# AlmondGod/diffusion-piano

Measured on AMD Instinct MI355X. Metric: env steps/sec at 4096 parallel envs; qpos L∞ drift vs CPU MuJoCo, higher is better.
Workload: dtype f32; 1 GPU; 4096 envs/GPU crossing_field random-action rollout, 10 physics substeps per env-step, constraint forces by the primal Newton solve (friction loss, uncapped rows); envs_per_gpu=4096, song=crossing_field, parallelism=dp1

## Files before the change

__graft_entry__.py:

```python

from __future__ import annotations

import importlib
import os
import subprocess
import sys
from pathlib import Path

ROOT = Path(__file__).resolve().parent
PKG = ROOT / "diffusion-piano_amd"
HIPCC = os.environ.get("HIPCC", "/opt/rocm/bin/hipcc")


_PENDING = []


def _hipcc(src_name, out_name, extra_deps=(), flags=(), wait=True):
    src = PKG / "csrc" / src_name
    out = PKG / out_name
    deps = [src, *extra_deps, Path(__file__)]
    if out.exists() and all(out.stat().st_mtime >= d.stat().st_mtime for d in deps):
        return out
    cmd = [HIPCC, "--offload-arch=gfx950", "-O3", "-std=c++17", "-fPIC", "-shared", "-Wno-unused-value", *flags,
           "-o", str(out), str(src)]
    if wait:
        subprocess.run(cmd, check=True)
    else:
        _PENDING.append((subprocess.Popen(cmd), cmd))
    return out


def _join():
    while _PENDING:
        proc, cmd = _PENDING.pop()
        if proc.wait() != 0:
            raise subprocess.CalledProcessError(proc.returncode, cmd)


def _hipcc_lib():
    csrc = PKG / "csrc"
    deps = [csrc / "devmodel.h", csrc / "prims.h", csrc / "collide_x.h", csrc / "kernel_v2.inc", csrc / "newton.inc",
            csrc / "augment.inc", csrc / "song_build.h", ROOT / "include" / "pianosim.h"]
    flags = ["-fno-hip-fp32-correctly-rounded-divide-sqrt", "-falign-loops=64", "-mllvm", "-amdgpu-sched-strategy=max-ilp"]
    out = _hipcc("pianosim.hip", "libpianosim.so", deps, flags=flags, wait=False)
    _hipcc("pianosim.hip", "libpianosim_timing.so", deps, flags=flags + ["-DPS_TIMING"], wait=False)
    return out


def _hipcc_xcheck():
    csrc = PKG / "csrc"
    src, out = ROOT / "tools" / "xcheck.hip", ROOT / "tools" / "libxcheck.so"
    deps = [src, csrc / "devmodel.h", csrc / "prims.h", csrc / "collide_x.h", ROOT / "include" / "pianosim.h"]
    if out.exists() and all(out.stat().st_mtime >= d.stat().st_mtime for d in deps):
        return out
    subprocess.run([HIPCC, "--offload-arch=gfx950", "-O3", "-std=c++17", "-fPIC", "-shared", "-Wno-unused-value",
                    "-fno-hip-fp32-correctly-rounded-divide-sqrt", "-o", str(out), str(src)], check=True)
    return out


def _hipcc_ldl_bench():
    src, out = ROOT / "tools" / "ldl_bench.hip", ROOT / "tools" / "libldlbench.so"
    if out.exists() and out.stat().st_mtime >= src.stat().st_mtime:
        return out
    subprocess.run([HIPCC, "--offload-arch=gfx950", "-O3", "-std=c++17", "-fPIC", "-shared", "-Wno-unused-value",
                    "-o", str(out), str(src)], check=True)
    return out


def _hipcc_rl():
    deps = [ROOT / "include" / "pianorl.h", PKG / "csrc" / "mlp_step.inc", PKG / "csrc" / "mlp_split.inc"]
    ilp = ["-mllvm", "-amdgpu-sched-strategy=max-ilp"]
    _hipcc("pianorl.hip", "libpianorl_timing.so", deps, flags=ilp + ["-DMLP_TIMING"], wait=False)
    return _hipcc("pianorl.hip", "libpianorl.so", deps, flags=ilp, wait=False)


def _gxx_song():
    src = PKG / "csrc" / "song.cpp"
    out = PKG / "libpianosong.so"
    deps = [src, PKG / "csrc" / "song_build.h", ROOT / "include" / "pianosong.h", Path(__file__)]
    if out.exists() and all(out.stat().st_mtime >= d.stat().st_mtime for d in deps):
        return out
    subprocess.run(["g++", "-O2", "-std=c++17", "-fPIC", "-shared", "-Wall", "-ffp-contract=off", "-o", str(out),
                    str(src)], check=True)
    return out


def build() -> None:
    _hipcc_lib()
    _hipcc_rl()
    _hipcc_xcheck()
    _hipcc_ldl_bench()
    _gxx_song()
    _join()
    subprocess.run(["make", "-s", "-C", str(ROOT / "oracle")], check=True)
    sys.path.insert(0, str(ROOT))
    pkg = importlib.import_module("diffusion-piano_amd")
    lib = importlib.import_module("diffusion-piano_amd._lib").load()
    assert lib.ps_model_desc_size() > 0
# ... 47 lines not shown
```

diffusion-piano_amd/csrc/kernel_v2.inc:

```

#ifdef PS_TIMING
#define NPHASE 56
#define TARG , uint64_t *tacc, uint64_t &tlast
#define TPASS , tacc, tlast
#define TSTAMP(slot)                                     \
  do {                                                   \
    __syncthreads();                                     \
    uint64_t t_ = __builtin_amdgcn_s_memtime();         \
    tacc[slot] += t_ - tlast;                            \
    tlast = t_;                                          \
  } while (0)
__device__ uint64_t* g_timing = nullptr;
#else
#define TSTAMP(slot) \
  do {               \
  } while (0)
#define TARG
#define TPASS
#endif

#ifdef PS_CHECK_A
__device__ int g_dbg_count = 0;
#endif
enum : int { BX_R = 0, BX_CP = 0, BX_O = 10, BX_W = 13, BX_AL = 16, BX_AC = 19, BX_F = 22, BX_N = 25, BXS = 28 };
// ... 1105 lines not shown
    float val;
    if (i < G) {
      int j = i / (NK + 1), k = i - j * (NK + 1);
      int t = t_obs + j;
      val = t < song.T ? song.goal[t * (NK + 1) + k] : 0.f;
    } else if (i < o_s) {
      int slot = i - o_f;
      val = 0.f;
      for (int n = 0; n < song.count[t_obs]; n++) {
        int f = song.fingers[t_obs * PS_MAX_NOTES + n];
        int idx = f < 5 ? (f < 0 ? f + 5 : f) : f;
        if (idx == slot) val = 1.f;
      }
    } else if (i < o_s + NK) {
      val = S.knorm[i - o_s];
    } else if (i == o_s + NK) {
      val = S.sustain;
    } else {
      val = S.dx[m->obs_dof[i - o_s - NK - 1]][6];
    }
    obs[i] = val;
  }
}

__device__ __forceinline__ void key_state2(const DevModel* __restrict__ m, Shared& S, const LaneDyn& D, int lane) {
  uint64_t bits[2];
#pragma unroll
  for (int j = 0; j < 2; j++) {
    int k = lane + 64 * j;
    bool act = false;
    if (k < NK) {
      float khi = m->key_hi[k];
      float s = clampf(D.kq[j], m->key_lo[k], khi);
      S.knorm[k] = s / khi;
      act = fabsf(s - khi) <= KEY_THRESHOLD;
    }
    bits[j] = __ballot(act);
  }
  if (lane == 0) {
    S.act_bits[0] = (int)(bits[0] & 0xffffffffull);
    S.act_bits[1] = (int)(bits[0] >> 32);
    S.act_bits[2] = (int)(bits[1] & 0xffffffull);
  }
  wsync();
}

#ifndef PS_BIG_SWEEPS
#define PS_BIG_SWEEPS 2
#endif
#ifndef PS_WAVES_PER_EU
#define PS_WAVES_PER_EU 2
#endif
#ifndef PS_CHUNKS
#define PS_CHUNKS 3
#endif
template <bool XG, int WPE, bool Q>
__device__ __forceinline__ bool env_step(Shared& S, const DevModel* __restrict__ m, const Song& songs, const Cfg& cfg,
                                         const Bufs& bufs, const float* __restrict__ action,
                                         const uint8_t* __restrict__ mask, float* __restrict__ obs,
                                         float* __restrict__ reward, float* __restrict__ discount,
                                         uint8_t* __restrict__ step_type, const int mode, const int e, const int lane,
                                         const int chunk, const int chunks) {
  const bool first = !Q || chunk == 0;
  const Song song = song_of(songs, e);
  float* obs_e = obs + (size_t)e * cfg.obs_dim;
  bool do_reset;
  if (mode == 1) {
    if (mask && !mask[e]) return false;
    do_reset = true;
  } else {
    do_reset = first && bufs.last[e] != 0;
  }
  const float* applied = bufs.applied ? bufs.applied + (size_t)e * NV : nullptr;
  const float* cw = bufs.park + (size_t)e * PARK_WORDS * 64 + lane;
  int cscal = 0;
  if (Q && !first) {
    cscal = __float_as_int(ld_wt(cw + 64 * CW_SCAL));
    if (__builtin_amdgcn_readlane(cscal, CS_NOAPPLIED)) applied = nullptr;
  }
  float hand_dy = 0.f;
  if (do_reset) {
    const int ep = bufs.episode[e];
    if (cfg.randomize) hand_dy = hand_offset_draw(cfg.seed_lo, cfg.seed_hi, (int)(cfg.env0 + (uint32_t)e), ep);
    if (lane == 0) {
      bufs.episode[e] = ep + 1;
      bufs.hand_dy[e] = hand_dy;
    }
  } else if (cfg.randomize) {
    hand_dy = bufs.hand_dy[e];
  }
  LaneStatic L;
  load_static(m, S, L, lane);
  LaneDyn D;
  const size_t rowoff = (size_t)e * NV;
  D.qws = 0.f;
#pragma unroll
  for (int j = 0; j < 2; j++) D.kws[j] = 0.f;
  if (do_reset) {
    D.q = D.v = 0.f;
    #pragma unroll
    for (int j = 0; j < 2; j++) { D.kq[j] = D.kv[j] = 0.f; }
    if (lane == 0) S.sustain = 0.f;
  } else if (Q && !first) {
    D.q = ld_wt(cw + 64 * CW_Q);
    D.v = ld_wt(cw + 64 * CW_V);
#pragma unroll
    for (int j = 0; j < 2; j++) {
// ... 23 lines not shown
    if (src < 0) ctrl = 0.f;
    if (Q && !first) ctrl = ld_wt(cw + 64 * CW_CTRL);
    const float sv = a_e[m->n_action - 1];
    if (lane == 0) S.sustain = cfg.canonical ? (sv + 1.f) * 0.5f : sv;
  }
  wsync();
  float actf_last = 0.f;
  int st_solves = 0, st_concap = 0, st_cap = 0, st_maxrow = 0, st_coupled = 0, st_piv = 0, st_cdofs = 0;
#ifdef PS_TIMING
  uint64_t tacc[NPHASE] = {0};
  uint64_t tlast = __builtin_amdgcn_s_memtime();
#endif
  int warn[PS_NWARN] = {0, 0, 0};
  if (Q && !first) {
    actf_last = ld_wt(cw + 64 * CW_ACTF);
    st_solves = __builtin_amdgcn_readlane(cscal, CS_SOLVES);
    st_concap = __builtin_amdgcn_readlane(cscal, CS_CONCAP);
    st_cap = __builtin_amdgcn_readlane(cscal, CS_CAP);
    st_maxrow = __builtin_amdgcn_readlane(cscal, CS_MAXROW);
    st_coupled = __builtin_amdgcn_readlane(cscal, CS_COUPLED);
    st_piv = __builtin_amdgcn_readlane(cscal, CS_PIV);
    st_cdofs = __builtin_amdgcn_readlane(cscal, CS_CDOFS);
    static_assert(PS_NWARN == 3, "carried warning counters");
    warn[0] = __builtin_amdgcn_readlane(cscal, CS_WARN);
    warn[1] = __builtin_amdgcn_readlane(cscal, CS_WARN + 1);
    warn[2] = __builtin_amdgcn_readlane(cscal, CS_WARN + 2);
  }
#define PS_RESET_PHYSICS()                                                              \
  do {                                                                                  \
    D.q = D.v = D.qws = 0.f;                                                            \
    for (int j_ = 0; j_ < 2; j_++) D.kq[j_] = D.kv[j_] = D.kws[j_] = 0.f;               \
    ctrl = 0.f;                                                                         \
    if (applied) {                                                                      \
      for (int i_ = lane; i_ < NV; i_ += 64) const_cast<float*>(applied)[i_] = 0.f;     \
      applied = nullptr;                                                                \
    }                                                                                   \
  } while (0)
  if (!do_reset) {
    bool acc_reset = false;
    NGuess guess;
    guess.zf = guess.zl = guess.zc = 0;
    guess.cid = -2;
    guess.zk[0] = guess.zk[1] = 0;
    guess.valid = false;
    if (Q && !first) {
      guess.zf = __float_as_int(ld_wt(cw + 64 * CW_ZF));
      guess.zl = __float_as_int(ld_wt(cw + 64 * CW_ZL));
      guess.zc = __float_as_int(ld_wt(cw + 64 * CW_ZC));
      guess.cid = __float_as_int(ld_wt(cw + 64 * CW_CID));
      guess.zk[0] = __float_as_int(ld_wt(cw + 64 * CW_ZK));
      guess.zk[1] = __float_as_int(ld_wt(cw + 64 * (CW_ZK + 1)));
      guess.valid = __builtin_amdgcn_readlane(cscal, CS_GVALID) != 0;
    }
    const int s_begin = Q ? chunk * m->nsub / chunks : 0;
    const int s_end = Q ? (chunk + 1) * m->nsub / chunks : m->nsub;
    for (int s = s_begin; s < (Q ? s_end : m->nsub); s++) {
      {
        bool bq = lane < NDT && !(fabsf(D.q) <= 1e10f), bv = false;
#pragma unroll
        for (int j = 0; j < 2; j++)
          if (lane + 64 * j < NK) bq |= !(fabsf(D.kq[j]) <= 1e10f);
        if (__ballot(bq)) { warn[PS_WARN_BADQPOS]++; PS_RESET_PHYSICS(); }
        bv = lane < NDT && !(fabsf(D.v) <= 1e10f);
#pragma unroll
        for (int j = 0; j < 2; j++)
          if (lane + 64 * j < NK) bv |= !(fabsf(D.kv[j]) <= 1e10f);
        if (__ballot(bv)) { warn[PS_WARN_BADQVEL]++; PS_RESET_PHYSICS(); }
      }
      int zoff = 0;
      asm volatile("" : "+s"(zoff));
      const DevModel* __restrict__ mq = m + zoff;
      int lq = lane;
      asm volatile("" : "+v"(lq));
      kinematics2<true, XG>(mq, S, L, D, lq, hand_dy TPASS);
      TSTAMP(0);
      D.actf = ctrl;
      dynamics2(mq, S, L, D, applied, lq TPASS);
      actf_last = D.w;
      TSTAMP(1);
      if (XG) {
        float* pkc = bufs.park + (size_t)e * PARK_WORDS * 64 + lq;
#pragma unroll
        for (int a = 0; a < MAXDEP; a++) {
          pkc[64 * a] = D.M[a];
          pkc[64 * (9 + a)] = D.Mh[a];
        }
        pkc[64 * 18] = D.q; pkc[64 * 19] = D.v; pkc[64 * 20] = D.qws; pkc[64 * 21] = D.qfs;
#pragma unroll
        for (int j = 0; j < 2; j++) {
          pkc[64 * (22 + j)] = D.kq[j];
          pkc[64 * (24 + j)] = D.kv[j];
          pkc[64 * (26 + j)] = D.kws[j];
          pkc[64 * (28 + j)] = D.kqfs[j];
        }
        asm volatile("" ::: "memory");
      }
      st_concap += collide2<XG, WPE>(mq, S, cfg.maxcon, lq, L.c_r TPASS) >= cfg.maxcon;
      if (XG) {
        asm volatile("" ::: "memory");
        const float* pkc = bufs.park + (size_t)e * PARK_WORDS * 64 + lq;
#pragma unroll
        for (int a = 0; a < MAXDEP; a++) {
          D.M[a] = pkc[64 * a];
          D.Mh[a] = pkc[64 * (9 + a)];
        }
        D.q = pkc[64 * 18]; D.v = pkc[64 * 19]; D.qws = pkc[64 * 20]; D.qfs = pkc[64 * 21];
#pragma unroll
        for (int j = 0; j < 2; j++) {
// ... 341 lines not shown
  if (lane == 0) {
    float* tm = bufs.terms + (size_t)e * PS_NTERMS;
    tm[0] = kp; tm[1] = sus; tm[2] = energy; tm[3] = fing; tm[4] = fore;
    reward[e] = kp + sus + energy + fing + fore;
    discount[e] = disc;
    step_type[e] = terminal ? PS_LAST : PS_MID;
    float* ma = bufs.mus_acc + (size_t)e * PS_NMUSIC;
#pragma unroll
    for (int i = 0; i < PS_NMUSIC; i++) ma[i] += mus[i];
    if (terminal) {
      float* me = bufs.mus_ep + (size_t)e * PS_NMUSIC;
      const float inv = 1.f / (float)t_new;
#pragma unroll
      for (int i = 0; i < PS_NMUSIC; i++) me[i] = ma[i] * inv;
      bufs.mus_cnt[e] += 1;
    }
    bufs.sustain[e] = S.sustain;
    bufs.t_idx[e] = t_new;
    bufs.last[e] = terminal ? 1 : 0;
    bufs.ncon[e] = S.ncon;
  }
  if (bufs.con_out) {
    constexpr int CW = (int)(sizeof(Contact) / sizeof(int));
    const int* src = reinterpret_cast<const int*>(S.con);
    int* dst = reinterpret_cast<int*>(bufs.con_out) + (size_t)e * MAXCON * CW;
    for (int w = lane; w < S.ncon * CW; w += 64) dst[w] = src[w];
  }
#ifdef PS_TIMING
  TSTAMP(5);
  if (lane == 0 && g_timing)
    for (int i = 0; i < NPHASE; i++) g_timing[(size_t)e * NPHASE + i] += tacc[i];
#endif
  return false;
}

template <bool XG, int WPE = PS_WAVES_PER_EU>
__global__ void __launch_bounds__(64) __attribute__((amdgpu_waves_per_eu(WPE))) pianosim_kernel(const DevModel* __restrict__ m, Song song, Cfg cfg, Bufs bufs,
                                                      const float* __restrict__ action, const uint8_t* __restrict__ mask,
                                                      float* __restrict__ obs, float* __restrict__ reward,
                                                      float* __restrict__ discount, uint8_t* __restrict__ step_type,
                                                      int mode, int n_envs, const int* __restrict__ order) {
#ifdef PS_DYN_LDS
  extern __shared__ __attribute__((aligned(16))) char smem_[];
  Shared& S = *reinterpret_cast<Shared*>(smem_);
#else
  __shared__ Shared S;
#endif
  const int e = order ? order[blockIdx.x] : (int)blockIdx.x;
  const int lane = threadIdx.x;
  if (e >= n_envs) return;
  env_step<XG, WPE, false>(S, m, song, cfg, bufs, action, mask, obs, reward, discount, step_type, mode, e, lane, 0, 1);
}

enum : int { QC_HEAD = 0, QC_TAIL = 32, QC_WORDS = 64 };
#ifndef PS_TIMING
enum : int { QE_NONE = -1, QE_LEFT = -2 };
struct QArgs {
  const DevModel* m;
  Song song;
  Cfg cfg;
  Bufs bufs;
  const float* action;
  float *obs, *reward, *discount;
  uint8_t* step_type;
  int n_envs;
  int *queue, *ctr;
  int cap, chunks;
};
template <bool XG>
__global__ void __launch_bounds__(64) __attribute__((amdgpu_waves_per_eu(PS_WAVES_PER_EU))) pianosim_queue_kernel(
    const QArgs ka) {
  __shared__ Shared S;
  typedef __attribute__((address_space(4))) const QArgs* KArgs;
  const uint64_t kbase = (uint64_t)__builtin_amdgcn_kernarg_segment_ptr();
  int own = ka.queue[blockIdx.x];
  for (;;) {
    int lane = threadIdx.x;
    asm volatile("" : "+v"(lane));
    uint64_t kp = kbase;
    asm volatile("" : "+s"(kp));
    const QArgs& a = *(const QArgs*)(KArgs)kp;
    int item = own;
    if (own < 0 && lane == 0) {
      const int t = __hip_atomic_fetch_add(&a.ctr[QC_HEAD], 1, __ATOMIC_RELAXED, __HIP_MEMORY_SCOPE_AGENT);
      if (t < a.cap) item = __hip_atomic_exchange(&a.queue[t], QE_LEFT, __ATOMIC_RELAXED, __HIP_MEMORY_SCOPE_AGENT);
      __builtin_amdgcn_fence(__ATOMIC_ACQUIRE, "agent");
    }
    asm volatile("s_waitcnt vmcnt(0)" ::: "memory");
    item = __builtin_amdgcn_readfirstlane(item);
    asm volatile("" : "+s"(item));
    wsync();
    if (item < 0) return;
    const int e = item >> 4, chunk = item & 15;
    if (e >= a.n_envs) return;
    const bool more = env_step<XG, PS_WAVES_PER_EU, true>(S, a.m, a.song, a.cfg, a.bufs, a.action, nullptr, a.obs, a.reward,
                                                          a.discount, a.step_type, 0, e, lane, chunk, a.chunks);
    asm volatile("s_waitcnt vmcnt(0)" ::: "memory");
    wsync();
    own = QE_NONE;
    if (more) {
      const int next = (e << 4) | (chunk + 1);
      int old = QE_NONE;
      if (lane == 0) {
        const int slot = __hip_atomic_fetch_add(&a.ctr[QC_TAIL], 1, __ATOMIC_RELAXED, __HIP_MEMORY_SCOPE_AGENT);
        old = slot < a.cap ? __hip_atomic_exchange(&a.queue[slot], next, __ATOMIC_RELAXED, __HIP_MEMORY_SCOPE_AGENT)
                           : (int)QE_LEFT;
      }
      if (__builtin_amdgcn_readfirstlane(old) == QE_LEFT) own = next;
    }
    wsync();
  }
}
#endif
```

diffusion-piano_amd/csrc/pianosim.hip:

```cpp
#include <hip/hip_runtime.h>
#include <math.h>
#include <stdint.h>
#include <stdio.h>
#include <stdlib.h>
#include <string.h>

#include <string>
#include <vector>

#include "devmodel.h"
#include "prims.h"
#include "collide_x.h"

using namespace ps;

#include "kernel_v2.inc"
#include "augment.inc"

static thread_local std::string g_err;
static int fail(const std::string& s) {
  g_err = s;
  return -1;
}
#define HIPCHK(x)                                                                    \
  do {                                                                               \
    hipError_t e_ = (x);                                                             \
    if (e_ != hipSuccess) return fail(std::string(#x) + ": " + hipGetErrorString(e_)); \
  } while (0)

struct ps_env {
  int n, device, obs_dim, action_dim;
  int64_t env_offset;
  int full_cpl;
  ps_task_cfg cfg;
  DevModel* d_model;
  int T;
  float* d_goal;
  int *d_count, *d_keys, *d_fingers;
  float *qpos, *qvel, *qws, *ctrl, *sustain, *applied, *terms, *tips;
  int *t_idx, *ncon;
  float *mus_acc, *mus_ep;
  int* mus_cnt;
  int* order;
  bool ordered;
  uint8_t* last;
  bool applied_on;
  float* hand_dy;
  int* episode;
  int* stats;
  int* warnings;
  float* park;
  uint64_t seed;
  bool has_x;
  int wave_slots;
  int chunks, step_grid;
  bool chunks_forced;
  int *queue, *qctr;
  Contact* con_out;
  bool aug_on;
  AugDev aug;
  size_t aug_lds;
  std::vector<void*> aug_mem;
};

struct DeviceGuard {
  int prev = -1;
  bool ok = true;
  explicit DeviceGuard(int dev) {
    if (hipGetDevice(&prev) != hipSuccess) prev = -1;
    if (prev != dev) ok = hipSetDevice(dev) == hipSuccess;
  }
  ~DeviceGuard() {
    int cur = -1;
    if (prev >= 0 && hipGetDevice(&cur) == hipSuccess && cur != prev) (void)hipSetDevice(prev);
  }
};
#define GUARD(E)                                                                  \
  DeviceGuard guard_((E)->device);                                                \
  if (!guard_.ok) return fail("hipSetDevice(" + std::to_string((E)->device) + ") failed")

static void quat2mat_h(const double* q, float* R) {
  double n = sqrt(q[0] * q[0] + q[1] * q[1] + q[2] * q[2] + q[3] * q[3]);
  double w = q[0] / n, x = q[1] / n, y = q[2] / n, z = q[3] / n;
  double M[9] = {1 - 2 * (y * y + z * z), 2 * (x * y - w * z), 2 * (x * z + w * y),
                 2 * (x * y + w * z), 1 - 2 * (x * x + z * z), 2 * (y * z - w * x),
                 2 * (x * z - w * y), 2 * (y * z + w * x), 1 - 2 * (x * x + y * y)};
  for (int i = 0; i < 9; i++) R[i] = (float)M[i];
}

static void enclosing_capsule(const double (*v)[3], int n, float* out) {
  double best = INFINITY;
  double lo[3] = {INFINITY, INFINITY, INFINITY}, hi[3] = {-INFINITY, -INFINITY, -INFINITY};
  for (int i = 0; i < n; i++)
    for (int k = 0; k < 3; k++) { lo[k] = fmin(lo[k], v[i][k]); hi[k] = fmax(hi[k], v[i][k]); }
  for (int a = 0; a < 3; a++) {
    const int b = (a + 1) % 3, c = (a + 2) % 3;
    const double cb = 0.5 * (lo[b] + hi[b]), cc = 0.5 * (lo[c] + hi[c]);
    double r = 0.0;
    for (int i = 0; i < n; i++) r = fmax(r, hypot(v[i][b] - cb, v[i][c] - cc));
    double t0 = INFINITY, t1 = -INFINITY;
    for (int i = 0; i < n; i++) {
      const double rho = hypot(v[i][b] - cb, v[i][c] - cc), s = sqrt(fmax(r * r - rho * rho, 0.0));
      t0 = fmin(t0, v[i][a] + s);
      t1 = fmax(t1, v[i][a] - s);
    }
    if (t0 > t1) t0 = t1 = 0.5 * (t0 + t1);
    const double vol = M_PI * r * r * (t1 - t0) + 4.0 / 3.0 * M_PI * r * r * r;
    if (vol < best) {
      best = vol;
      double p0[3], p1[3];
// ... 359 lines not shown
    for (int s = 0; s < PS_NFINGER; s++) {
      m->site_body[h * PS_NFINGER + s] = h * NB + d->site_body[h][s];
      for (int i = 0; i < 3; i++) m->site_pos[h * PS_NFINGER + s][i] = (float)d->site_pos[h][s][i];
    }
  if (d->n_cappairs < 0 || d->n_cappairs > PS_MAX_CAPPAIRS) return fail("bad n_cappairs");
  m->npairs = d->n_cappairs;
  for (int i = 0; i < d->n_cappairs; i++) {
    m->pair[i][0] = d->cappair[i][0];
    m->pair[i][1] = d->cappair[i][1];
    if (m->pair[i][0] < 0 || m->pair[i][0] >= NGT || m->pair[i][1] < 0 || m->pair[i][1] >= NGT)
      return fail("capsule pair index out of range");
    if (m->geom_r[m->pair[i][0]] < 0.f || m->geom_r[m->pair[i][1]] < 0.f) return fail("capsule pair names an unused slot");
  }
  m->npairs_same = 0;
  while (m->npairs_same < m->npairs && m->pair[m->npairs_same][0] / NG == m->pair[m->npairs_same][1] / NG)
    m->npairs_same++;
  for (int i = m->npairs_same; i < m->npairs; i++)
    if (m->pair[i][0] / NG == m->pair[i][1] / NG) { m->npairs_same = m->npairs; break; }
  auto xhand = [](int g) { return g < NGT ? g / NG : (g - NGT) / NX; };
  m->nxpairs_same = 0;
  while (m->nxpairs_same < m->nxpairs &&
         xhand(m->xpair[m->nxpairs_same] & 255) == xhand(m->xpair[m->nxpairs_same] >> 8))
    m->nxpairs_same++;
  for (int i = m->nxpairs_same; i < m->nxpairs; i++)
    if (xhand(m->xpair[i] & 255) == xhand(m->xpair[i] >> 8)) { m->nxpairs_same = m->nxpairs; break; }
  return 0;
}

static void free_aug(ps_env* E) {
  for (void* p : E->aug_mem) (void)hipFree(p);
  E->aug_mem.clear();
  E->aug_on = false;
}

static int launch_builder(ps_env* E, int mode, const uint8_t* mask, const int* f_song, const double* f_factor,
                          const int* f_shift, void* stream) {
  hipLaunchKernelGGL(song_build_kernel, dim3(E->n), dim3(64), E->aug_lds, (hipStream_t)stream, E->aug, mode, mask,
                     E->last, E->episode, (uint32_t)E->seed, (uint32_t)(E->seed >> 32), (uint32_t)E->env_offset, E->n,
                     f_song, f_factor, f_shift);
  HIPCHK(hipGetLastError());
  return 0;
}

extern "C" {

const char* ps_last_error(void) { return g_err.c_str(); }
int ps_version(void) { return 4; }
int ps_model_desc_size(void) { return (int)sizeof(ps_model_desc); }
int ps_obs_dim(const ps_task_cfg* cfg) {
  if (!cfg || cfg->struct_size != PS_TASK_CFG_SIZE)
    return fail("ps_task_cfg.struct_size != sizeof(ps_task_cfg): rebuild against include/pianosim.h");
  return (cfg->n_steps_lookahead + 1) * (NK + 1) + (cfg->fingering_reward ? 10 : 0) + NK + 1 + NH * ND;
}

int ps_create(const ps_model_desc* model, const ps_song_desc* song, const ps_task_cfg* cfg, int n_envs, int device,
              uint64_t seed, ps_env** out) {
  if (!model || !song || !cfg || !out) return fail("null argument");
  if (cfg->struct_size != PS_TASK_CFG_SIZE)
    return fail("ps_task_cfg.struct_size != sizeof(ps_task_cfg): rebuild against include/pianosim.h");
  if (n_envs <= 0) return fail("n_envs must be positive");
  if (song->T <= 0) return fail("empty song");
  if (cfg->n_steps_lookahead < 0) return fail("negative lookahead");
  if (cfg->max_contacts < 0 || cfg->max_contacts > MAXCON) return fail("max_contacts out of range");
  if (cfg->solver_iterations < 0) return fail("negative solver_iterations");
  if (cfg->solver_refine < 0 || cfg->solver_refine > 2) return fail("solver_refine must be 0, 1 or 2");
  if (cfg->solver != PS_SOLVER_NEWTON) return fail("unknown solver (PS_SOLVER_NEWTON is the only one)");
  for (int t = 0; t < song->T; t++) {
    if (song->count[t] < 0 || song->count[t] > PS_MAX_NOTES) return fail("bad note count");
    int k = 0;
    for (int j = 0; j < NK; j++) k += song->goal[(size_t)t * (NK + 1) + j] != 0.f;
    if (k > PS_MAX_NOTES)
      return fail("step " + std::to_string(t) + " has " + std::to_string(k) + " goal keys; at most " +
                  std::to_string(PS_MAX_NOTES) + " are supported");
  }
  DeviceGuard guard_(device);
  if (!guard_.ok) return fail("hipSetDevice(" + std::to_string(device) + ") failed");
  DevModel* hm = new DevModel;
  if (build_dev_model(model, hm)) { delete hm; return -1; }
  const bool has_x = hm->nx > 0 || hm->nxpairs > 0;
  ps_env* E = new ps_env();
  E->n = n_envs;
  E->device = device;
  E->cfg = *cfg;
  E->obs_dim = ps_obs_dim(cfg) - NH * ND + hm->n_obsj;
  E->action_dim = hm->n_action;
  E->has_x = has_x;
  E->T = song->T;
  size_t N = (size_t)n_envs;
  HIPCHK(hipMalloc(&E->d_model, sizeof(DevModel)));
  HIPCHK(hipMemcpy(E->d_model, hm, sizeof(DevModel), hipMemcpyHostToDevice));
  delete hm;
  HIPCHK(hipMalloc(&E->d_goal, sizeof(float) * song->T * (NK + 1)));
  HIPCHK(hipMemcpy(E->d_goal, song->goal, sizeof(float) * song->T * (NK + 1), hipMemcpyHostToDevice));
  HIPCHK(hipMalloc(&E->d_count, sizeof(int) * song->T));
  HIPCHK(hipMemcpy(E->d_count, song->count, sizeof(int) * song->T, hipMemcpyHostToDevice));
  HIPCHK(hipMalloc(&E->d_keys, sizeof(int) * song->T * PS_MAX_NOTES));
  HIPCHK(hipMemcpy(E->d_keys, song->keys, sizeof(int) * song->T * PS_MAX_NOTES, hipMemcpyHostToDevice));
  HIPCHK(hipMalloc(&E->d_fingers, sizeof(int) * song->T * PS_MAX_NOTES));
  HIPCHK(hipMemcpy(E->d_fingers, song->fingers, sizeof(int) * song->T * PS_MAX_NOTES, hipMemcpyHostToDevice));
  HIPCHK(hipMalloc(&E->qpos, sizeof(float) * N * NV));
  HIPCHK(hipMalloc(&E->qvel, sizeof(float) * N * NV));
  HIPCHK(hipMalloc(&E->qws, sizeof(float) * N * NV));
  HIPCHK(hipMalloc(&E->applied, sizeof(float) * N * NV));
  HIPCHK(hipMalloc(&E->ctrl, sizeof(float) * N * NU));
  HIPCHK(hipMalloc(&E->sustain, sizeof(float) * N));
  HIPCHK(hipMalloc(&E->terms, sizeof(float) * N * PS_NTERMS));
// ... 4 lines not shown
  HIPCHK(hipMalloc(&E->mus_ep, sizeof(float) * N * PS_NMUSIC));
  HIPCHK(hipMalloc(&E->mus_cnt, sizeof(int) * N));
  HIPCHK(hipMalloc(&E->order, sizeof(int) * N));
  HIPCHK(hipMalloc(&E->last, N));
  HIPCHK(hipMalloc(&E->hand_dy, sizeof(float) * N));
  HIPCHK(hipMalloc(&E->episode, sizeof(int) * N));
  HIPCHK(hipMalloc(&E->stats, sizeof(int) * N * PS_NSTATS));
  HIPCHK(hipMalloc(&E->warnings, sizeof(int) * N * PS_NWARN));
  HIPCHK(hipMemset(E->warnings, 0, sizeof(int) * N * PS_NWARN));
  HIPCHK(hipMalloc(&E->park, sizeof(float) * N * PARK_WORDS * 64));
  HIPCHK(hipMemset(E->hand_dy, 0, sizeof(float) * N));
  HIPCHK(hipMemset(E->episode, 0, sizeof(int) * N));
  HIPCHK(hipMemset(E->stats, 0, sizeof(int) * N * PS_NSTATS));
  E->seed = seed;
  E->env_offset = 0;
  HIPCHK(hipMemset(E->qpos, 0, sizeof(float) * N * NV));
  HIPCHK(hipMemset(E->qvel, 0, sizeof(float) * N * NV));
  HIPCHK(hipMemset(E->qws, 0, sizeof(float) * N * NV));
  HIPCHK(hipMemset(E->applied, 0, sizeof(float) * N * NV));
  HIPCHK(hipMemset(E->ctrl, 0, sizeof(float) * N * NU));
  HIPCHK(hipMemset(E->sustain, 0, sizeof(float) * N));
  HIPCHK(hipMemset(E->terms, 0, sizeof(float) * N * PS_NTERMS));
  HIPCHK(hipMemset(E->tips, 0, sizeof(float) * N * 2 * PS_NFINGER * 3));
  HIPCHK(hipMemset(E->t_idx, 0, sizeof(int) * N));
  HIPCHK(hipMemset(E->ncon, 0, sizeof(int) * N));
  HIPCHK(hipMemset(E->mus_acc, 0, sizeof(float) * N * PS_NMUSIC));
  HIPCHK(hipMemset(E->mus_ep, 0, sizeof(float) * N * PS_NMUSIC));
  HIPCHK(hipMemset(E->mus_cnt, 0, sizeof(int) * N));
  HIPCHK(hipMemset(E->last, 0, N));
  HIPCHK(hipDeviceSynchronize());
  E->applied_on = false;
  E->ordered = !(getenv("PIANOSIM_NO_ORDER") && atoi(getenv("PIANOSIM_NO_ORDER")));
  E->full_cpl = getenv("PIANOSIM_DEBUG_FULL_COUPLED") && atoi(getenv("PIANOSIM_DEBUG_FULL_COUPLED"));
  {
    int cus = 0;
    HIPCHK(hipDeviceGetAttribute(&cus, hipDeviceAttributeMultiprocessorCount, device));
    E->wave_slots = 4 * cus;
    const char* w = getenv("PIANOSIM_ONE_WAVE_MAX");
    if (w) E->wave_slots = atoi(w);
    const char* c = getenv("PIANOSIM_CHUNKS");
    E->chunks_forced = c != nullptr;
    E->chunks = c ? atoi(c) : PS_CHUNKS;
    if (E->chunks > PS_MAX_CHUNKS) E->chunks = PS_MAX_CHUNKS;
    if (E->chunks > model->n_substeps) E->chunks = model->n_substeps;
    if (E->chunks < 2) E->chunks = 0;
    const char* g = getenv("PIANOSIM_STEP_GRID");
    E->step_grid = g && atoi(g) > 0 ? atoi(g) : PS_WAVES_PER_EU * 4 * cus;
#ifdef PS_TIMING
    E->chunks = 0;
#endif
    if (E->chunks) {
      HIPCHK(hipMalloc(&E->queue, sizeof(int) * N * E->chunks));
      HIPCHK(hipMalloc(&E->qctr, sizeof(int) * QC_WORDS));
    }
  }
  *out = E;
  return 0;
}

int ps_env_obs_dim(const ps_env* E) { return E ? E->obs_dim : fail("null env"); }
int ps_env_action_dim(const ps_env* E) { return E ? E->action_dim : fail("null env"); }

void ps_destroy(ps_env* E) {
  if (!E) return;
  DeviceGuard guard_(E->device);
  hipFree(E->d_model); hipFree(E->d_goal); hipFree(E->d_count); hipFree(E->d_keys); hipFree(E->d_fingers);
  hipFree(E->qpos); hipFree(E->qvel); hipFree(E->qws); hipFree(E->applied); hipFree(E->ctrl); hipFree(E->sustain);
  hipFree(E->terms); hipFree(E->tips); hipFree(E->t_idx); hipFree(E->ncon); hipFree(E->last);
  hipFree(E->mus_acc); hipFree(E->mus_ep); hipFree(E->mus_cnt); hipFree(E->order);
  hipFree(E->hand_dy); hipFree(E->episode); hipFree(E->stats); hipFree(E->warnings); hipFree(E->park);
  if (E->con_out) hipFree(E->con_out);
  if (E->queue) hipFree(E->queue);
  if (E->qctr) hipFree(E->qctr);
  free_aug(E);
  delete E;
}

#ifdef PS_DYN_LDS
#define PS_LAUNCH_LDS PS_DYN_LDS
#else
#define PS_LAUNCH_LDS 0
#endif
constexpr int ORDER_THREADS = 1024;
constexpr int ORDER_BUCKETS = 130;
__global__ void __launch_bounds__(ORDER_THREADS) order_kernel(const int* __restrict__ stats,
                                                              const uint8_t* __restrict__ last,
                                                              int* __restrict__ order, int n, int* __restrict__ queue,
                                                              int* __restrict__ qctr, int qcap, int qhead,
                                                              bool sorted) {
  __shared__ int hist[ORDER_BUCKETS], base[ORDER_BUCKETS];
  if (queue) {
    for (int i = n + threadIdx.x; i < qcap; i += blockDim.x) queue[i] = -1;
    if (threadIdx.x == 0) {
      qctr[QC_HEAD] = qhead;
      qctr[QC_TAIL] = n;
    }
    if (!sorted) {
      for (int e = threadIdx.x; e < n; e += blockDim.x) queue[e] = e << 4;
      return;
    }
  }
  if (threadIdx.x < ORDER_BUCKETS) hist[threadIdx.x] = 0;
  __syncthreads();
  for (int e = threadIdx.x; e < n; e += blockDim.x) {
    const int b = last[e] ? 0 : 1 + min(max(stats[(size_t)e * PS_NSTATS + PS_STAT_SOLVES], 0), 128);
    atomicAdd(&hist[b], 1);
  }
  __syncthreads();
  if (threadIdx.x == 0) {
    int acc = 0;
    for (int b = ORDER_BUCKETS - 1; b >= 0; b--) {
      base[b] = acc;
      acc += hist[b];
    }
  }
  __syncthreads();
  for (int e = threadIdx.x; e < n; e += blockDim.x) {
    const int b = last[e] ? 0 : 1 + min(max(stats[(size_t)e * PS_NSTATS + PS_STAT_SOLVES], 0), 128);
    const int pos = atomicAdd(&base[b], 1);
    if (queue) queue[pos] = e << 4;
    else order[pos] = e;
  }
}

static int launch(ps_env* E, int mode, const float* action, const uint8_t* mask, float* obs, float* reward,
                  float* discount, uint8_t* step_type, void* stream) {
  Song song{E->T, E->d_goal, E->d_count, E->d_keys, E->d_fingers, 0, nullptr};
  if (E->aug_on) {
    song = Song{E->T, E->aug.goal, E->aug.count, E->aug.keys, E->aug.fingers, E->aug.T_cap, E->aug.T};
    if (launch_builder(E, mode == 1 ? AUG_RESET : AUG_STEP, mask, nullptr, nullptr, nullptr, stream)) return -1;
  }
  Cfg cfg{E->cfg.n_steps_lookahead, E->cfg.fingering_reward, E->cfg.forearm_reward, E->cfg.wrong_press_termination,
          E->cfg.solver_iterations, E->cfg.max_contacts, E->obs_dim, E->cfg.canonical_actions,
          (float)E->cfg.energy_penalty_coef, E->cfg.randomize_hand_positions != 0,
          (uint32_t)E->seed, (uint32_t)(E->seed >> 32), (uint32_t)E->env_offset, E->full_cpl,
          E->cfg.solver_refine};
  Bufs b{E->qpos, E->qvel, E->qws, E->ctrl, E->sustain, E->t_idx, E->last,
         E->applied_on ? E->applied : nullptr, E->terms, E->tips, E->ncon, E->mus_acc, E->mus_ep, E->mus_cnt,
         E->hand_dy, E->episode, E->stats, E->con_out, E->warnings, E->park};
  const bool sliced = mode == 0 && E->chunks >= 2 && (E->chunks_forced || E->n > E->step_grid);
  if (sliced) {
    const int cap = E->n * E->chunks, grid = E->n < E->step_grid ? E->n : E->step_grid;
    hipLaunchKernelGGL(order_kernel, dim3(1), dim3(ORDER_THREADS), 0, (hipStream_t)stream, E->stats, E->last, E->order,
                       E->n, E->queue, E->qctr, cap, grid, E->ordered);
    HIPCHK(hipGetLastError());
#ifndef PS_TIMING
    const QArgs qa{E->d_model, song, cfg, b, action, obs, reward, discount, step_type, E->n, E->queue, E->qctr, cap,
                   E->chunks};
#define PS_LAUNCH_Q(XG)                                                                                           \
  hipLaunchKernelGGL((pianosim_queue_kernel<XG>), dim3(grid), dim3(64), 0, (hipStream_t)stream, qa)
    if (E->has_x) PS_LAUNCH_Q(true); else PS_LAUNCH_Q(false);
#undef PS_LAUNCH_Q
#endif
    HIPCHK(hipGetLastError());
    return 0;
  }
  const int* order = nullptr;
  if (mode == 0 && E->ordered && E->n >= 2048) {
    hipLaunchKernelGGL(order_kernel, dim3(1), dim3(ORDER_THREADS), 0, (hipStream_t)stream, E->stats, E->last, E->order,
                       E->n, (int*)nullptr, (int*)nullptr, 0, 0, true);
    HIPCHK(hipGetLastError());
    order = E->order;
  }
  const bool one = E->n <= E->wave_slots;
#define PS_LAUNCH(XG, WPE)                                                                                    \
  hipLaunchKernelGGL((pianosim_kernel<XG, WPE>), dim3(E->n), dim3(64), PS_LAUNCH_LDS, (hipStream_t)stream, \
                     E->d_model, song, cfg, b, action, mask, obs, reward, discount, step_type, mode, E->n, order)
  if (E->has_x) {
    if (one) PS_LAUNCH(true, 1); else PS_LAUNCH(true, PS_WAVES_PER_EU);
  } else {
    if (one) PS_LAUNCH(false, 1); else PS_LAUNCH(false, PS_WAVES_PER_EU);
  }
#undef PS_LAUNCH
  HIPCHK(hipGetLastError());
  return 0;
}

int ps_reset(ps_env* E, const uint8_t* env_mask, float* obs, void* stream) {
  if (!E || !obs) return fail("null argument");
  GUARD(E);
  return launch(E, 1, nullptr, env_mask, obs, nullptr, nullptr, nullptr, stream);
}

int ps_step(ps_env* E, const float* action, float* obs, float* reward, float* discount, uint8_t* step_type,
            void* stream) {
  if (!E || !action || !obs || !reward || !discount || !step_type) return fail("null argument");
  GUARD(E);
  return launch(E, 0, action, nullptr, obs, reward, discount, step_type, stream);
}

int ps_get_state(ps_env* E, float* qpos, float* qvel, float* qacc_ws, float* ctrl, float* sustain, int32_t* t_idx,
                 uint8_t* last, void* stream) {
  if (!E) return fail("null env");
  GUARD(E);
  hipStream_t s = (hipStream_t)stream;
  size_t N = E->n;
  if (qpos) HIPCHK(hipMemcpyAsync(qpos, E->qpos, sizeof(float) * N * NV, hipMemcpyDeviceToDevice, s));
  if (qvel) HIPCHK(hipMemcpyAsync(qvel, E->qvel, sizeof(float) * N * NV, hipMemcpyDeviceToDevice, s));
  if (qacc_ws) HIPCHK(hipMemcpyAsync(qacc_ws, E->qws, sizeof(float) * N * NV, hipMemcpyDeviceToDevice, s));
  if (ctrl) HIPCHK(hipMemcpyAsync(ctrl, E->ctrl, sizeof(float) * N * NU, hipMemcpyDeviceToDevice, s));
  if (sustain) HIPCHK(hipMemcpyAsync(sustain, E->sustain, sizeof(float) * N, hipMemcpyDeviceToDevice, s));
  if (t_idx) HIPCHK(hipMemcpyAsync(t_idx, E->t_idx, sizeof(int) * N, hipMemcpyDeviceToDevice, s));
  if (last) HIPCHK(hipMemcpyAsync(last, E->last, N, hipMemcpyDeviceToDevice, s));
  return 0;
}

int ps_set_state(ps_env* E, const float* qpos, const float* qvel, const float* qacc_ws, const float* ctrl,
                 const float* sustain, const int32_t* t_idx, const uint8_t* last, void* stream) {
  if (!E) return fail("null env");
  GUARD(E);
  hipStream_t s = (hipStream_t)stream;
  size_t N = E->n;
  if (qpos) HIPCHK(hipMemcpyAsync(E->qpos, qpos, sizeof(float) * N * NV, hipMemcpyDeviceToDevice, s));
// ... 1 lines not shown
  if (qacc_ws) HIPCHK(hipMemcpyAsync(E->qws, qacc_ws, sizeof(float) * N * NV, hipMemcpyDeviceToDevice, s));
  if (ctrl) HIPCHK(hipMemcpyAsync(E->ctrl, ctrl, sizeof(float) * N * NU, hipMemcpyDeviceToDevice, s));
  if (sustain) HIPCHK(hipMemcpyAsync(E->sustain, sustain, sizeof(float) * N, hipMemcpyDeviceToDevice, s));
  if (t_idx) HIPCHK(hipMemcpyAsync(E->t_idx, t_idx, sizeof(int) * N, hipMemcpyDeviceToDevice, s));
  if (last) HIPCHK(hipMemcpyAsync(E->last, last, N, hipMemcpyDeviceToDevice, s));
  return 0;
}

int ps_set_applied(ps_env* E, const float* qfrc_applied, void* stream) {
  if (!E) return fail("null env");
  GUARD(E);
  if (!qfrc_applied) {
    E->applied_on = false;
    return 0;
  }
  HIPCHK(hipMemcpyAsync(E->applied, qfrc_applied, sizeof(float) * E->n * NV, hipMemcpyDeviceToDevice,
                        (hipStream_t)stream));
  E->applied_on = true;
  return 0;
}

int ps_reward_terms(ps_env* E, float* terms, void* stream) {
  if (!E || !terms) return fail("null argument");
  GUARD(E);
  HIPCHK(hipMemcpyAsync(terms, E->terms, sizeof(float) * E->n * PS_NTERMS, hipMemcpyDeviceToDevice,
                        (hipStream_t)stream));
  return 0;
}

int ps_fingertips(ps_env* E, float* xpos, void* stream) {
  if (!E || !xpos) return fail("null argument");
  GUARD(E);
  HIPCHK(hipMemcpyAsync(xpos, E->tips, sizeof(float) * E->n * 2 * PS_NFINGER * 3, hipMemcpyDeviceToDevice,
                        (hipStream_t)stream));
  return 0;
}

#ifdef PS_TIMING
int ps_debug_timing(ps_env* E, uint64_t* out) {
  static uint64_t* d = nullptr;
  static size_t cap = 0;
  size_t bytes = sizeof(uint64_t) * E->n * NPHASE;
  if (cap < bytes) {
    if (d) (void)hipFree(d);
    HIPCHK(hipMalloc(&d, bytes));
    cap = bytes;
    HIPCHK(hipMemset(d, 0, bytes));
    HIPCHK(hipMemcpyToSymbol(HIP_SYMBOL(g_timing), &d, sizeof(d)));
    return 0;
  }
  HIPCHK(hipDeviceSynchronize());
  if (out) HIPCHK(hipMemcpy(out, d, bytes, hipMemcpyDeviceToHost));
  HIPCHK(hipMemset(d, 0, bytes));
  return 0;
}
#endif

int ps_musical_metrics(ps_env* E, float* episode, int32_t* episodes, void* stream) {
  if (!E) return fail("null argument");
  GUARD(E);
  if (episode)
    HIPCHK(hipMemcpyAsync(episode, E->mus_ep, sizeof(float) * E->n * PS_NMUSIC, hipMemcpyDeviceToDevice,
                          (hipStream_t)stream));
  if (episodes)
    HIPCHK(hipMemcpyAsync(episodes, E->mus_cnt, sizeof(int) * E->n, hipMemcpyDeviceToDevice, (hipStream_t)stream));
  return 0;
}

int ps_solver_stats(ps_env* E, int32_t* stats, void* stream) {
  if (!E || !stats) return fail("null argument");
  GUARD(E);
  HIPCHK(hipMemcpyAsync(stats, E->stats, sizeof(int) * E->n * PS_NSTATS, hipMemcpyDeviceToDevice, (hipStream_t)stream));
  return 0;
}

int ps_get_hand_offset(ps_env* E, float* dy, int32_t* episodes, void* stream) {
  if (!E) return fail("null argument");
  GUARD(E);
  if (dy) HIPCHK(hipMemcpyAsync(dy, E->hand_dy, sizeof(float) * E->n, hipMemcpyDeviceToDevice, (hipStream_t)stream));
  if (episodes)
    HIPCHK(hipMemcpyAsync(episodes, E->episode, sizeof(int) * E->n, hipMemcpyDeviceToDevice, (hipStream_t)stream));
  return 0;
}

int ps_set_hand_offset(ps_env* E, const float* dy, void* stream) {
  if (!E || !dy) return fail("null argument");
  GUARD(E);
  if (!E->cfg.randomize_hand_positions) return fail("ps_set_hand_offset needs randomize_hand_positions");
  HIPCHK(hipMemcpyAsync(E->hand_dy, dy, sizeof(float) * E->n, hipMemcpyDeviceToDevice, (hipStream_t)stream));
  return 0;
}

static_assert(sizeof(ps_contact) == sizeof(Contact), "ps_contact mirrors the kernel's contact record");
int ps_record_contacts(ps_env* E, int on) {
  if (!E) return fail("null argument");
  GUARD(E);
  if (on && !E->con_out) {
    HIPCHK(hipMalloc(&E->con_out, sizeof(Contact) * MAXCON * (size_t)E->n));
    HIPCHK(hipMemset(E->con_out, 0, sizeof(Contact) * MAXCON * (size_t)E->n));
  } else if (!on && E->con_out) {
    HIPCHK(hipFree(E->con_out));
    E->con_out = nullptr;
  }
  return 0;
}

// ... 228 lines not shown
```

Before: 861,700 env-steps/s.

## Place continuation chunks at fixed ranked queue slots and raise chunk count

```diff
diff --git a/__graft_entry__.py b/__graft_entry__.py
--- a/__graft_entry__.py
+++ b/__graft_entry__.py
@@ -44,6 +44,7 @@
     flags = ["-fno-hip-fp32-correctly-rounded-divide-sqrt", "-falign-loops=64", "-mllvm", "-amdgpu-sched-strategy=max-ilp"]
     out = _hipcc("pianosim.hip", "libpianosim.so", deps, flags=flags, wait=False)
     _hipcc("pianosim.hip", "libpianosim_timing.so", deps, flags=flags + ["-DPS_TIMING"], wait=False)
+    _hipcc("pianosim.hip", "libpianosim_qtrace.so", deps, flags=flags + ["-DPS_QTRACE"], wait=False)
     return out
 
 
diff --git a/diffusion-piano_amd/csrc/kernel_v2.inc b/diffusion-piano_amd/csrc/kernel_v2.inc
--- a/diffusion-piano_amd/csrc/kernel_v2.inc
+++ b/diffusion-piano_amd/csrc/kernel_v2.inc
@@ -1181,7 +1181,7 @@
 #define PS_WAVES_PER_EU 2
 #endif
 #ifndef PS_CHUNKS
-#define PS_CHUNKS 3
+#define PS_CHUNKS 6
 #endif
 template <bool XG, int WPE, bool Q>
 __device__ __forceinline__ bool env_step(Shared& S, const DevModel* __restrict__ m, const Song& songs, const Cfg& cfg,
@@ -1311,8 +1311,9 @@
       guess.zk[1] = __float_as_int(ld_wt(cw + 64 * (CW_ZK + 1)));
       guess.valid = __builtin_amdgcn_readlane(cscal, CS_GVALID) != 0;
     }
-    const int s_begin = Q ? chunk * m->nsub / chunks : 0;
-    const int s_end = Q ? (chunk + 1) * m->nsub / chunks : m->nsub;
+    const int s_each = Q ? m->nsub / chunks : 0, s_more = Q ? m->nsub - s_each * chunks : 0;
+    const int s_begin = Q ? chunk * s_each + min(chunk, s_more) : 0;
+    const int s_end = Q ? (chunk + 1) * s_each + min(chunk + 1, s_more) : m->nsub;
     for (int s = s_begin; s < (Q ? s_end : m->nsub); s++) {
       {
         bool bq = lane < NDT && !(fabsf(D.q) <= 1e10f), bv = false;
@@ -1760,7 +1761,7 @@
   env_step<XG, WPE, false>(S, m, song, cfg, bufs, action, mask, obs, reward, discount, step_type, mode, e, lane, 0, 1);
 }
 
-enum : int { QC_HEAD = 0, QC_TAIL = 32, QC_WORDS = 64 };
+enum : int { QC_HEAD = 0, QC_WORDS = 32 };
 #ifndef PS_TIMING
 enum : int { QE_NONE = -1, QE_LEFT = -2 };
 struct QArgs {
@@ -1774,7 +1775,17 @@
   int n_envs;
   int *queue, *ctr;
   int cap, chunks;
+  const int* rank;
+#ifdef PS_QTRACE
+  unsigned long long* trace;
+#endif
 };
+enum : int { QT_ITEM = 4, QT_EXIT = 2 };
+#ifdef PS_QTRACE
+#define QT(...) __VA_ARGS__
+#else
+#define QT(...)
+#endif
 template <bool XG>
 __global__ void __launch_bounds__(64) __attribute__((amdgpu_waves_per_eu(PS_WAVES_PER_EU))) pianosim_queue_kernel(
     const QArgs ka) {
@@ -1789,30 +1800,48 @@
     asm volatile("" : "+s"(kp));
     const QArgs& a = *(const QArgs*)(KArgs)kp;
     int item = own;
+    QT(const unsigned long long qt_turn = __builtin_amdgcn_s_memrealtime(); int qt_ticket = -1;)
     if (own < 0 && lane == 0) {
-      const int t = __hip_atomic_fetch_add(&a.ctr[QC_HEAD], 1, __ATOMIC_RELAXED, __HIP_MEMORY_SCOPE_AGENT);
-      if (t < a.cap) item = __hip_atomic_exchange(&a.queue[t], QE_LEFT, __ATOMIC_RELAXED, __HIP_MEMORY_SCOPE_AGENT);
+      for (;;) {
+        const int t = __hip_atomic_fetch_add(&a.ctr[QC_HEAD], 1, __ATOMIC_RELAXED, __HIP_MEMORY_SCOPE_AGENT);
+        QT(qt_ticket = t;)
+        if (t >= a.cap) break;
+        item = __hip_atomic_exchange(&a.queue[t], QE_LEFT, __ATOMIC_RELAXED, __HIP_MEMORY_SCOPE_AGENT);
+        if (item >= 0) break;
+        QT(a.trace[(size_t)a.cap * QT_ITEM + blockIdx.x * QT_EXIT + 1] += 1;)
+      }
       __builtin_amdgcn_fence(__ATOMIC_ACQUIRE, "agent");
     }
     asm volatile("s_waitcnt vmcnt(0)" ::: "memory");
     item = __builtin_amdgcn_readfirstlane(item);
     asm volatile("" : "+s"(item));
     wsync();
-    if (item < 0) return;
+    if (item < 0) {
+      QT(if (lane == 0) a.trace[(size_t)a.cap * QT_ITEM + blockIdx.x * QT_EXIT] = __builtin_amdgcn_s_memrealtime();)
+      return;
+    }
     const int e = item >> 4, chunk = item & 15;
     if (e >= a.n_envs) return;
+    QT(if (lane == 0) {
+      unsigned long long* rec = a.trace + ((size_t)chunk * a.n_envs + e) * QT_ITEM;
+      rec[0] = qt_turn;
+      rec[1] = __builtin_amdgcn_s_memrealtime();
+      rec[3] = (unsigned long long)(unsigned)qt_ticket << 32 | blockIdx.x;
+    })
     const bool more = env_step<XG, PS_WAVES_PER_EU, true>(S, a.m, a.song, a.cfg, a.bufs, a.action, nullptr, a.obs, a.reward,
                                                           a.discount, a.step_type, 0, e, lane, chunk, a.chunks);
     asm volatile("s_waitcnt vmcnt(0)" ::: "memory");
     wsync();
+    QT(if (lane == 0) a.trace[((size_t)chunk * a.n_envs + e) * QT_ITEM + 2] = __builtin_amdgcn_s_memrealtime();)
     own = QE_NONE;
     if (more) {
       const int next = (e << 4) | (chunk + 1);
       int old = QE_NONE;
       if (lane == 0) {
-        const int slot = __hip_atomic_fetch_add(&a.ctr[QC_TAIL], 1, __ATOMIC_RELAXED, __HIP_MEMORY_SCOPE_AGENT);
-        old = slot < a.cap ? __hip_atomic_exchange(&a.queue[slot], next, __ATOMIC_RELAXED, __HIP_MEMORY_SCOPE_AGENT)
-                           : (int)QE_LEFT;
+        const int slot = (chunk + 1) * a.n_envs + a.rank[e];
+        old = (unsigned)slot < (unsigned)a.cap
+                  ? __hip_atomic_exchange(&a.queue[slot], next, __ATOMIC_RELAXED, __HIP_MEMORY_SCOPE_AGENT)
+                  : (int)QE_LEFT;
       }
       if (__builtin_amdgcn_readfirstlane(old) == QE_LEFT) own = next;
     }
diff --git a/diffusion-piano_amd/csrc/pianosim.hip b/diffusion-piano_amd/csrc/pianosim.hip
--- a/diffusion-piano_amd/csrc/pianosim.hip
+++ b/diffusion-piano_amd/csrc/pianosim.hip
@@ -56,6 +56,8 @@
   int chunks, step_grid;
   bool chunks_forced;
   int *queue, *qctr;
+  int* qrank;
+  uint64_t* qtrace;
   Contact* con_out;
   bool aug_on;
   AugDev aug;
@@ -521,6 +523,13 @@
     return fail("ps_task_cfg.struct_size != sizeof(ps_task_cfg): rebuild against include/pianosim.h");
   return (cfg->n_steps_lookahead + 1) * (NK + 1) + (cfg->fingering_reward ? 10 : 0) + NK + 1 + NH * ND;
 }
+
+#ifdef PS_QTRACE
+static int qtrace_grid(const ps_env* E) { return E->n < E->step_grid ? E->n : E->step_grid; }
+static size_t qtrace_bytes(const ps_env* E) {
+  return sizeof(uint64_t) * ((size_t)E->n * E->chunks * QT_ITEM + (size_t)qtrace_grid(E) * QT_EXIT);
+}
+#endif
 
 int ps_create(const ps_model_desc* model, const ps_song_desc* song, const ps_task_cfg* cfg, int n_envs, int device,
               uint64_t seed, ps_env** out) {
@@ -631,6 +640,10 @@
     if (E->chunks) {
       HIPCHK(hipMalloc(&E->queue, sizeof(int) * N * E->chunks));
       HIPCHK(hipMalloc(&E->qctr, sizeof(int) * QC_WORDS));
+      HIPCHK(hipMalloc(&E->qrank, sizeof(int) * N));
+#ifdef PS_QTRACE
+      HIPCHK(hipMalloc(&E->qtrace, qtrace_bytes(E)));
+#endif
     }
   }
   *out = E;
@@ -651,6 +664,8 @@
   if (E->con_out) hipFree(E->con_out);
   if (E->queue) hipFree(E->queue);
   if (E->qctr) hipFree(E->qctr);
+  if (E->qrank) hipFree(E->qrank);
+  if (E->qtrace) hipFree(E->qtrace);
   free_aug(E);
   delete E;
 }
@@ -666,16 +681,16 @@
                                                               const uint8_t* __restrict__ last,
                                                               int* __restrict__ order, int n, int* __restrict__ queue,
                                                               int* __restrict__ qctr, int qcap, int qhead,
-                                                              bool sorted) {
+                                                              bool sorted, int* __restrict__ qrank) {
   __shared__ int hist[ORDER_BUCKETS], base[ORDER_BUCKETS];
   if (queue) {
     for (int i = n + threadIdx.x; i < qcap; i += blockDim.x) queue[i] = -1;
-    if (threadIdx.x == 0) {
-      qctr[QC_HEAD] = qhead;
-      qctr[QC_TAIL] = n;
-    }
+    if (threadIdx.x == 0) qctr[QC_HEAD] = qhead;
     if (!sorted) {
-      for (int e = threadIdx.x; e < n; e += blockDim.x) queue[e] = e << 4;
+      for (int e = threadIdx.x; e < n; e += blockDim.x) {
+        queue[e] = e << 4;
+        qrank[e] = e;
+      }
       return;
     }
   }
@@ -697,8 +712,12 @@
   for (int e = threadIdx.x; e < n; e += blockDim.x) {
     const int b = last[e] ? 0 : 1 + min(max(stats[(size_t)e * PS_NSTATS + PS_STAT_SOLVES], 0), 128);
     const int pos = atomicAdd(&base[b], 1);
-    if (queue) queue[pos] = e << 4;
-    else order[pos] = e;
+    if (queue) {
+      queue[pos] = e << 4;
+      qrank[e] = pos;
+    } else {
+      order[pos] = e;
+    }
   }
 }
 
@@ -721,11 +740,17 @@
   if (sliced) {
     const int cap = E->n * E->chunks, grid = E->n < E->step_grid ? E->n : E->step_grid;
     hipLaunchKernelGGL(order_kernel, dim3(1), dim3(ORDER_THREADS), 0, (hipStream_t)stream, E->stats, E->last, E->order,
-                       E->n, E->queue, E->qctr, cap, grid, E->ordered);
+                       E->n, E->queue, E->qctr, cap, grid, E->ordered, E->qrank);
     HIPCHK(hipGetLastError());
 #ifndef PS_TIMING
+#ifdef PS_QTRACE
+    HIPCHK(hipMemsetAsync(E->qtrace, 0, qtrace_bytes(E), (hipStream_t)stream));
     const QArgs qa{E->d_model, song, cfg, b, action, obs, reward, discount, step_type, E->n, E->queue, E->qctr, cap,
-                   E->chunks};
+                   E->chunks, E->qrank, (unsigned long long*)E->qtrace};
+#else
+    const QArgs qa{E->d_model, song, cfg, b, action, obs, reward, discount, step_type, E->n, E->queue, E->qctr, cap,
+                   E->chunks, E->qrank};
+#endif
 #define PS_LAUNCH_Q(XG)                                                                                           \
   hipLaunchKernelGGL((pianosim_queue_kernel<XG>), dim3(grid), dim3(64), 0, (hipStream_t)stream, qa)
     if (E->has_x) PS_LAUNCH_Q(true); else PS_LAUNCH_Q(false);
@@ -737,7 +762,7 @@
   const int* order = nullptr;
   if (mode == 0 && E->ordered && E->n >= 2048) {
     hipLaunchKernelGGL(order_kernel, dim3(1), dim3(ORDER_THREADS), 0, (hipStream_t)stream, E->stats, E->last, E->order,
-                       E->n, (int*)nullptr, (int*)nullptr, 0, 0, true);
+                       E->n, (int*)nullptr, (int*)nullptr, 0, 0, true, (int*)nullptr);
     HIPCHK(hipGetLastError());
     order = E->order;
   }
@@ -845,6 +870,21 @@
   HIPCHK(hipDeviceSynchronize());
   if (out) HIPCHK(hipMemcpy(out, d, bytes, hipMemcpyDeviceToHost));
   HIPCHK(hipMemset(d, 0, bytes));
+  return 0;
+}
+#endif
+
+#ifdef PS_QTRACE
+int ps_debug_qtrace(ps_env* E, int32_t* dims, uint64_t* items, uint64_t* exits, int32_t* rank) {
+  if (!E || !E->qtrace) return fail("no time-sliced step in this handle");
+  GUARD(E);
+  HIPCHK(hipDeviceSynchronize());
+  const size_t ni = (size_t)E->n * E->chunks * QT_ITEM;
+  if (dims) dims[0] = E->chunks, dims[1] = qtrace_grid(E);
+  if (items) HIPCHK(hipMemcpy(items, E->qtrace, sizeof(uint64_t) * ni, hipMemcpyDeviceToHost));
+  if (exits)
+    HIPCHK(hipMemcpy(exits, E->qtrace + ni, sizeof(uint64_t) * qtrace_grid(E) * QT_EXIT, hipMemcpyDeviceToHost));
+  if (rank) HIPCHK(hipMemcpy(rank, E->qrank, sizeof(int) * E->n, hipMemcpyDeviceToHost));
   return 0;
 }
 #endif
```

After: 948,500 env-steps/s (median of 6 runs). 1.1x the previous value.
